# PRBonn/SHINE_mapping

Hardware: NVIDIA H100
Metric: sdf_train_points_per_sec_fwd_bwd (higher is better)
Workload: dtype f32

## Files before the change

shine_mapping_b200/csrc/shine_b200.cu:

```cuda

#include <cuda_runtime.h>
#include <math.h>
#include <stdint.h>

#include "shine_b200.h"

#ifndef SHINE_SECTOR_PROBE_TRAIN
#define SHINE_SECTOR_PROBE_TRAIN 0
#endif
#ifndef SHINE_SECTOR_PROBE_INFER
#define SHINE_SECTOR_PROBE_INFER 1
#endif
#ifndef SHINE_CPASYNC_PREFETCH
#define SHINE_CPASYNC_PREFETCH 0
#endif
#ifndef SHINE_GATHER_GROUP
#define SHINE_GATHER_GROUP 2
#endif
#ifndef SHINE_SLOT_PREFETCH
#define SHINE_SLOT_PREFETCH 0
#endif
#ifndef SHINE_ZERO_TILE_SKIP
#define SHINE_ZERO_TILE_SKIP 1
#endif
// ... 246 lines not shown
    const float s0 = odd ? v[0] : v[2], s1 = odd ? v[1] : v[3];
    const float r0 = __shfl_xor_sync(kFull, s0, 1), r1 = __shfl_xor_sync(kFull, s1, 1);
    if (!odd) { a[0] = v[0]; a[2] = v[1]; a[1] = r0; a[3] = r1; }
    else      { a[0] = r0;   a[2] = r1;   a[1] = v[2]; a[3] = v[3]; }
}
__device__ __forceinline__ void from_cfrag(const float (&c)[4], int odd, float (&v)[4]) {
    const float s0 = odd ? c[0] : c[2], s1 = odd ? c[1] : c[3];
    const float r0 = __shfl_xor_sync(kFull, s0, 1), r1 = __shfl_xor_sync(kFull, s1, 1);
    if (!odd) { v[0] = c[0]; v[1] = c[1]; v[2] = r0; v[3] = r1; }
    else      { v[0] = r0;   v[1] = r1;   v[2] = c[2]; v[3] = c[3]; }
}

#define SHINE_ACC_DECL float dW2[2][4][4], dW1[2][4], db2p[4][2], db1p[4][2], dw3p[4][2]

__device__ __forceinline__ float reduce_scatter_g8(const float (&v)[8], int lane) {
    float a[4], b[2];
    const bool b4 = (lane & 16) != 0, b3 = (lane & 8) != 0, b2 = (lane & 4) != 0;
#pragma unroll
    for (int i = 0; i < 4; ++i) a[i] = (b4 ? v[4 + i] : v[i]) + __shfl_xor_sync(kFull, b4 ? v[i] : v[4 + i], 16);
#pragma unroll
    for (int i = 0; i < 2; ++i) b[i] = (b3 ? a[2 + i] : a[i]) + __shfl_xor_sync(kFull, b3 ? a[i] : a[2 + i], 8);
    return (b2 ? b[1] : b[0]) + __shfl_xor_sync(kFull, b2 ? b[0] : b[1], 4);
}
__device__ __forceinline__ void round_bar(int id) { asm volatile("bar.sync %0, 128;" ::"r"(id) : "memory"); }

__device__ __forceinline__ int frag_chunk(int lane) { return lane ^ ((lane >> 2) & 6); }
template <int NTF>
__device__ __forceinline__ void load_afrag(const float* blk, int c, AFrag<NTF>& a) {
    const float4 v = *reinterpret_cast<const float4*>(blk + 4 * c);
    a.set_packed(v.x, v.y, v.z, v.w);
}
__device__ __forceinline__ void load_bfrag(const float* blk, int c, uint2& bh, uint2& bl) {
    const float2 v = *reinterpret_cast<const float2*>(blk + 2 * c);
    split_fast2(v.x, v.y, bh.x, bh.y, bl.x, bl.y);
}
__device__ __forceinline__ void stage_afrags(float* blk, const int (&sq)[2], const float (&c)[4][4]) {
#pragma unroll
    for (int mt = 0; mt < 2; ++mt)
#pragma unroll
        for (int q = 0; q < 2; ++q)
            *reinterpret_cast<float4*>(blk + 128 * mt + 4 * sq[q]) = make_float4(c[2 * mt][q], c[2 * mt + 1][q], c[2 * mt][2 + q], c[2 * mt + 1][2 + q]);
}
__device__ __forceinline__ int xfrag_word(int ks, int c) { return 64 * ks + 2 * (c ^ (8 * ks)); }
__device__ __forceinline__ void load_xfrag(const float* sx, int ks, int c, uint2& bh, uint2& bl) {
    const float2 v = *reinterpret_cast<const float2*>(sx + xfrag_word(ks, c));
    split_fast2(v.x, v.y, bh.x, bh.y, bl.x, bl.y);
}


constexpr int kGatherGroup = SHINE_GATHER_GROUP;

using shine_internal::StepParams;

struct SmemPlan {
    static constexpr int W1 = 0;
    static constexpr int W1T = W1 + 2 * kH * kF;
    static constexpr int W2 = W1T + 2 * kF * kWS;
    static constexpr int W2T = W2 + 2 * kH * kWS;
    static constexpr int B1 = W2T + 2 * kH * kWS;
    static constexpr int B2 = B1 + kH;
    static constexpr int W3 = B2 + kH;
    static constexpr int B3 = W3 + kH;
    static constexpr int GSCALE = B3 + 1;
    static constexpr int kDecGradFloats = kH * kF + kH + kH * kH + kH + kH + 1;
    static constexpr int RND = B3 + 4;
    static constexpr int PRE = RND + 8;
    static constexpr int kPrePerWarp = 5 * kTile;
    static constexpr int STAGE = PRE + 8 * kPrePerWarp;
    static constexpr int SA2 = 0;
    static constexpr int SB2 = SA2 + kTile * kH;
    static constexpr int SA1 = SB2 + kTile * kH;
    static constexpr int SX = SA1 + kTile * kH;
    static constexpr int kStagePerWarp = SX + kTile * kF;
    static constexpr int kGroupPerLevel = 4 * kTile;
};

constexpr int kMaxGroupedRuns = 6;

__device__ __forceinline__ void red_add_f2(float* p, float a, float b) {
    asm volatile("red.global.add.v2.f32 [%0], {%1,%2};" ::"l"(p), "f"(a), "f"(b) : "memory");
}
__device__ __forceinline__ int group_slot(int p) { return 4 * (p & 3) + (p >> 2); }

template <int LMAX>
__device__ __forceinline__ void grouped_scatter(const StepParams& P, int L, int tile, const float* __restrict__ pt,
                                                float* __restrict__ dtile, const float (&dxc)[4], int lane) {
    const int g = lane >> 2, t = lane & 3;
    *reinterpret_cast<float2*>(dtile + g * kF + 2 * t) = make_float2(dxc[0], dxc[1]);
    *reinterpret_cast<float2*>(dtile + (g + 8) * kF + 2 * t) = make_float2(dxc[2], dxc[3]);
    __syncwarp();
    uint2 bh[2], bl[2];
#pragma unroll
    for (int c = 0; c < 2; ++c)
        split_fast2(dtile[(8 * c + t) * kF + g], dtile[(8 * c + t + 4) * kF + g], bh[c].x, bh[c].y, bl[c].x, bl[c].y);
    const float sx = (g & 4) ? 1.f : -1.f, ox = (g & 4) ? 0.f : 1.f;
    const float sy = (g & 2) ? 1.f : -1.f, oy = (g & 2) ? 0.f : 1.f;
    const float sz = (g & 1) ? 1.f : -1.f, oz = (g & 1) ? 0.f : 1.f;
// ... 65 lines not shown
            a0.set(rid[0] == r ? w[0] : 0.f, rid[0] == r + 1 ? w[0] : 0.f, rid[1] == r ? w[1] : 0.f, rid[1] == r + 1 ? w[1] : 0.f);
            a1.set(rid[2] == r ? w[2] : 0.f, rid[2] == r + 1 ? w[2] : 0.f, rid[3] == r ? w[3] : 0.f, rid[3] == r + 1 ? w[3] : 0.f);
            float c0[4] = {0.f, 0.f, 0.f, 0.f}, c1[4] = {0.f, 0.f, 0.f, 0.f};
            mma3x2<3>(c0, c1, a0, a1, bh[0], bl[0], bh[1], bl[1]);
            if (v1 >= 0) {
                const int row = __ldg(slot_words + 16 * (int64_t)v1 + id_off);
                red_add_f2(gb + (int64_t)row * kF + 2 * t, c0[0] + c1[0], c0[1] + c1[1]);
            }
            if (v2 >= 0) {
                const int row = __ldg(slot_words + 16 * (int64_t)v2 + id_off);
                red_add_f2(gb + (int64_t)row * kF + 2 * t, c0[2] + c1[2], c0[3] + c1[3]);
            }
        }
    }
    __syncwarp();
}

template <int NTF, bool TRAIN, bool DEC_GRAD, int LMAX, bool GROUPED = false>
__global__ void __launch_bounds__(256, !TRAIN ? SHINE_INFER_MINB : (DEC_GRAD && !GROUPED) ? SHINE_TRAIN_DECGRAD_MINB : SHINE_TRAIN_MINB)
sdf_fused_kernel(const __grid_constant__ StepParams P) {
    static_assert(!GROUPED || TRAIN, "the grouped scatter belongs to the training kernels");
    static_assert(!DEC_GRAD || TRAIN, "decoder gradients belong to the training kernels");
    static_assert(SmemPlan::kStagePerWarp >= SmemPlan::kDecGradFloats, "a warp's staging area holds its partial decoder gradient");
    extern __shared__ __align__(16) float smem[];
    uint32_t* smu = reinterpret_cast<uint32_t*>(smem);
    const int tid = threadIdx.x, lane = tid & 31, warp = tid >> 5;
    const int g = lane >> 2, t = lane & 3, odd = t & 1, half = t >> 1;
    constexpr int kWarps = 8;

    for (int i = tid; i < kH * kF; i += blockDim.x) {
        const int nrow = i / kF, k = i % kF;
        uint32_t hi, lo; split_tf32(P.dec.w1[i], hi, lo);
        smu[SmemPlan::W1 + i] = hi; smu[SmemPlan::W1 + kH * kF + i] = lo;
        smu[SmemPlan::W1T + k * kWS + nrow] = hi; smu[SmemPlan::W1T + kF * kWS + k * kWS + nrow] = lo;
    }
    for (int i = tid; i < kH * kH; i += blockDim.x) {
        const int nrow = i / kH, k = i % kH;
        uint32_t hi, lo; split_tf32(P.dec.w2[i], hi, lo);
        smu[SmemPlan::W2 + nrow * kWS + k] = hi; smu[SmemPlan::W2 + kH * kWS + nrow * kWS + k] = lo;
        smu[SmemPlan::W2T + k * kWS + nrow] = hi; smu[SmemPlan::W2T + kH * kWS + k * kWS + nrow] = lo;
    }
    if (tid < kH) {
        smem[SmemPlan::B1 + tid] = P.dec.b1 ? P.dec.b1[tid] : 0.f;
        smem[SmemPlan::B2 + tid] = P.dec.b2 ? P.dec.b2[tid] : 0.f;
        smem[SmemPlan::W3 + tid] = P.dec.w3[tid];
    }
    if (tid == 0) {
        smem[SmemPlan::B3] = P.dec.b3 ? P.dec.b3[0] : 0.f;
        smem[SmemPlan::GSCALE] = P.loss_scale * ((TRAIN && P.d_loss) ? __ldg(P.d_loss) : 1.0f);
    }
    constexpr int kPark = LMAX <= 4 ? 16 : 32;
    constexpr int kIdPark = 4 * LMAX;
    __syncthreads();
    SHINE_ACC_DECL;
#pragma unroll
    for (int a = 0; a < 2; ++a) {
#pragma unroll
        for (int b = 0; b < 4; ++b) { dW2[a][b][0] = dW2[a][b][1] = dW2[a][b][2] = dW2[a][b][3] = 0.f; }
        dW1[a][0] = dW1[a][1] = dW1[a][2] = dW1[a][3] = 0.f;
    }
#pragma unroll
    for (int j = 0; j < 4; ++j) { db2p[j][0] = db2p[j][1] = db1p[j][0] = db1p[j][1] = dw3p[j][0] = dw3p[j][1] = 0.f; }
    float dW2acc[2][4] = {{0.f, 0.f, 0.f, 0.f}, {0.f, 0.f, 0.f, 0.f}}, dW1acc[4] = {0.f, 0.f, 0.f, 0.f};
    float dw3acc = 0.f, db2acc[2] = {0.f, 0.f}, db1acc[2] = {0.f, 0.f};
    constexpr bool kRounds = DEC_GRAD && GROUPED;

    constexpr bool kSectorProbe = TRAIN ? (SHINE_SECTOR_PROBE_TRAIN != 0) : (SHINE_SECTOR_PROBE_INFER != 0);
    constexpr bool kSlotPrefetch = TRAIN && !kSectorProbe && (SHINE_SLOT_PREFETCH != 0) && (SHINE_CPASYNC_PREFETCH == 0);
    constexpr bool kZeroSkip = (SHINE_ZERO_TILE_SKIP != 0) && (SHINE_CPASYNC_PREFETCH == 0);
    const bool poly = P.oct.poly_interp != 0;
    const int L = P.oct.num_levels;

    float db3p = 0.f;
    float loss_acc = 0.f;

    float* stage = smem + SmemPlan::STAGE + warp * SmemPlan::kStagePerWarp;
    float* stX = stage + SmemPlan::SX;
    const int kp = g >> 2, fc = frag_chunk(lane);
    const int sq[2] = {frag_chunk(8 * t + (g & 3)), frag_chunk(8 * t + 4 + (g & 3))};
    float* gpt = smem + SmemPlan::STAGE + (DEC_GRAD ? 8 * SmemPlan::kStagePerWarp : 0) +
                 warp * (LMAX * SmemPlan::kGroupPerLevel + (DEC_GRAD ? 0 : kTile * kF));
    float* gdx = DEC_GRAD ? stX : gpt + LMAX * SmemPlan::kGroupPerLevel;

    auto wgrad_round = [&](bool staged) {
        if (lane == 0) smu[SmemPlan::RND + warp] = staged ? 1u : 0u;
        round_bar(1 + 2 * (threadIdx.x >> 7));
        uint32_t present = 0;
#pragma unroll
        for (int v = 0; v < kWarps; ++v) present |= (smu[SmemPlan::RND + v] != 0u ? 1u : 0u) << v;
        const int mt = warp & 1, np = (warp >> 1) & 1, kh = warp >> 2;
#pragma unroll
        for (int i = 0; i < kWarps / 2; ++i) {
            const int v = 4 * kh + i;
            if (!((present >> v) & 1u)) continue;
            const float* s = smem + SmemPlan::STAGE + v * SmemPlan::kStagePerWarp;
#pragma unroll
            for (int ks = 0; ks < 2; ++ks) {
                uint2 bh[2], bl[2];
#pragma unroll
                for (int n = 0; n < 2; ++n) load_bfrag(s + SmemPlan::SB2 + (4 * ks + 2 * np + n) * 64, fc, bh[n], bl[n]);
                AFrag<NTF> a;
                const float4 av = *reinterpret_cast<const float4*>(s + SmemPlan::SA2 + (2 * ks + mt) * 128 + 4 * fc);
                a.set_packed(av.x, av.y, av.z, av.w);
                if (np == 0) { db2acc[0] += av.x + av.z; db2acc[1] += av.y + av.w; }
                mma3x2<NTF>(dW2acc[0], dW2acc[1], a, a, bh[0], bl[0], bh[1], bl[1]);
            }
        }
#pragma unroll
        for (int vv = 0; vv < 2; ++vv) {
            const int v = 2 * (warp >> 1) + vv;
            if (!((present >> v) & 1u)) continue;
            const float* s = smem + SmemPlan::STAGE + v * SmemPlan::kStagePerWarp;
#pragma unroll
            for (int ks = 0; ks < 2; ++ks) {
                uint2 bh, bl;
                load_xfrag(s + SmemPlan::SX, ks, fc, bh, bl);
                AFrag<NTF> a;
                const float4 av = *reinterpret_cast<const float4*>(s + SmemPlan::SA1 + (2 * ks + mt) * 128 + 4 * fc);
                a.set_packed(av.x, av.y, av.z, av.w);
                db1acc[0] += av.x + av.z; db1acc[1] += av.y + av.w;
                mma3<NTF>(dW1acc, a, bh, bl);
            }
        }
        round_bar(2 + 2 * (threadIdx.x >> 7));
    };

    const int warp_global = blockIdx.x * kWarps + warp;
    const int warp_stride = gridDim.x * kWarps;

    bool consecutive = true;
#pragma unroll
    for (int i = 1; i < LMAX; ++i)
        if (i < L && P.oct.lv[i].level != P.oct.lv[0].level - i) consecutive = false;

    unsigned long long skey0 = 0ull;
    int smine[LMAX / 2];
    uint4 skf[LMAX / 2];
#pragma unroll
    for (int j = 0; j < LMAX / 2; ++j) smine[j] = -1;
    auto stage_slots = [&](bool v, float sx, float sy, float sz) {
        skey0 = v ? morton_of(sx, sy, sz, P.oct.lv[0].level) : 0ull;
#pragma unroll
        for (int j = 0; j < LMAX / 2; ++j) {
            const int i = 2 * j + half;
            smine[j] = -1;
            if (i < L && v) {
                const shine_level& lv = P.oct.lv[i];
                const unsigned long long kq = consecutive ? (skey0 >> (3 * i)) : morton_of(sx, sy, sz, lv.level);
// ... 18 lines not shown

#if SHINE_CPASYNC_PREFETCH
    float* pre = smem + SmemPlan::PRE + warp * SmemPlan::kPrePerWarp;
    const uint32_t pre_s = (uint32_t)__cvta_generic_to_shared(pre);
    auto prefetch_inputs = [&](int tl) {
        if (tl < P.num_tiles) {
            const int64_t base = (int64_t)tl * kTile;
            const int64_t left = P.n - base;
            const int npts = left < kTile ? (int)left : kTile;
#pragma unroll
            for (int r = 0; r < 3; ++r) {
                const int wd = lane + 32 * r;
                const float* src = nullptr;
                if (wd < 48) { if (wd < 3 * npts) src = P.coord + 3 * base + wd; }
                else if (wd < 64) { if (P.label && wd - 48 < npts) src = P.label + base + (wd - 48); }
                else if (wd < 80) { if (P.weighted && wd - 64 < npts) src = P.weight + base + (wd - 64); }
                if (src) asm volatile("cp.async.ca.shared.global [%0], [%1], 4;" ::"r"(pre_s + 4u * (uint32_t)wd), "l"(src) : "memory");
            }
        }
        asm volatile("cp.async.commit_group;" ::: "memory");
    };
    prefetch_inputs(warp_global);

    for (int tile = warp_global; tile - (kRounds ? warp : 0) < P.num_tiles; tile += warp_stride) {
        const int64_t base = (int64_t)tile * kTile;
        const int64_t myp = base + g + 8 * odd;
        asm volatile("cp.async.wait_group 0;" ::: "memory");
        __syncwarp();
        const bool valid = myp < P.n;
        float x = 0.f, y = 0.f, z = 0.f, lab = 0.f, wgt = 1.f;
        if (valid) {
            const int lp = g + 8 * odd;
            x = pre[3 * lp]; y = pre[3 * lp + 1]; z = pre[3 * lp + 2];
            if (P.label) lab = pre[48 + lp];
            if (P.weighted) wgt = fabsf(pre[64 + lp]);
        }
        __syncwarp();
        prefetch_inputs(tile + warp_stride);

#else
    float nx = 0.f, ny = 0.f, nz = 0.f, nlab = 0.f, nwgt = 1.f;
    bool nvalid = false;
    auto prefetch_inputs = [&](int tl) {
        const int64_t p = (int64_t)tile_of(tl) * kTile + g + 8 * odd;
        nvalid = tl < P.num_tiles && p < P.n;
        if (nvalid) {
            nx = __ldg(P.coord + 3 * p); ny = __ldg(P.coord + 3 * p + 1); nz = __ldg(P.coord + 3 * p + 2);
            if (P.label) nlab = __ldg(P.label + p);
            if (P.weighted) nwgt = fabsf(__ldg(P.weight + p));
        }
    };
    prefetch_inputs(warp_global);
    if (kSlotPrefetch) stage_slots(nvalid, nx, ny, nz);

    int phase = kZeroSkip ? 0 : 1;
    bool advance = false, last_pass = false;
    float pred0 = 0.f, zsum = 0.f;
    auto bce_point = [&](float pv, float lb, float wg, float& li, float& dp) {
        const float zt = __fdividef(1.0f, 1.0f + __expf(-__fdividef(lb, P.sigma)));
        const float e = __expf(-fabsf(pv));
        li = fmaxf(pv, 0.f) - pv * zt + __logf(1.0f + e);
        dp = 0.f;
        if (TRAIN) {
            const float rs = __fdividef(1.0f, 1.0f + e);
            const float sg = pv >= 0.f ? rs : e * rs;
            dp = (sg - zt) * wg * smem[SmemPlan::GSCALE];
        }
    };
    const bool dynamic = (SHINE_DYNAMIC_TILES != 0) && !kRounds && P.tile_counter != nullptr;
    int next_tile = 0, pending = 0;
    if (dynamic && lane == 0) pending = atomicAdd(P.tile_counter, 1);
    for (int seq = warp_global;; seq = !advance ? seq : (dynamic ? next_tile : seq + warp_stride)) {
        if (last_pass) break;
        const int tile = tile_of(seq);
        if (phase == 1 && seq - (kRounds ? warp : 0) >= P.num_tiles) {
            if constexpr (kZeroSkip && DEC_GRAD) {
#pragma unroll
                for (int o = 16; o > 0; o >>= 1) zsum += __shfl_xor_sync(kFull, zsum, o);
                if (lane == 0) smem[SmemPlan::PRE + warp] = zsum;
                __syncthreads();
                if (!kRounds && warp != 0) break;
                float tot = 0.f;
#pragma unroll
                for (int w = 0; w < kWarps; ++w) tot += smem[SmemPlan::PRE + w];
                if (tot == 0.f) break;
                zsum = tot;
                phase = 2;
            } else {
                break;
            }
        }
        const bool virt = phase != 1;
        last_pass = phase == 2;
        advance = !virt;
        if (kRounds && phase == 2 && warp != 0) { wgrad_round(false); continue; }
        const int64_t base = (int64_t)tile * kTile;
        const int64_t myp = base + g + 8 * odd;
        const bool valid = virt ? false : nvalid;
        const float x = nx, y = ny, z = nz, lab = nlab, wgt = nwgt;
        if (!virt) {
            if (dynamic) {
                next_tile = warp_stride + __shfl_sync(kFull, pending, 0);
                prefetch_inputs(next_tile);
                if (lane == 0) pending = atomicAdd(P.tile_counter, 1);
            } else {
                prefetch_inputs(seq + warp_stride);
            }
        }

#endif
        float feat[4];
        float pk[kPark];
        float idp[kIdPark];
        uint32_t hitmask = 0;
        if constexpr (kSectorProbe) {
        {
            float acc[8] = {0.f, 0.f, 0.f, 0.f, 0.f, 0.f, 0.f, 0.f};
#pragma unroll
// ... 123 lines not shown
                    const float wz = half ? b.tz : b.uz;
                    const float w0 = __fmul_rn(__fmul_rn(b.ux, b.uy), wz), w1 = __fmul_rn(__fmul_rn(b.ux, b.ty), wz);
                    const float w2 = __fmul_rn(__fmul_rn(b.tx, b.uy), wz), w3 = __fmul_rn(__fmul_rn(b.tx, b.ty), wz);
                    blend4(acc, r0, r1, r2, r3, w0, w1, w2, w3);
                }
            }
#pragma unroll
            for (int q = 0; q < 4; ++q) {
                const float send = half ? acc[q] : acc[4 + q];
                const float recv = __shfl_xor_sync(kFull, send, 2);
                feat[q] = (half ? acc[4 + q] : acc[q]) + recv;
            }
        }
        }
#if !SHINE_CPASYNC_PREFETCH
        if (kZeroSkip && phase == 1 && __ballot_sync(kFull, hitmask != 0u) == 0u) {
            if (!TRAIN && P.mask && half == 0 && valid) P.mask[myp] = 0;
            if (P.pred && half == 0 && valid) P.pred[myp] = pred0;
            if (P.label != nullptr && valid) {
                float li, dpz;
                bce_point(pred0, lab, wgt, li, dpz);
                if (half == 0) { loss_acc += wgt * li; zsum += dpz; }
            }
            if (kRounds) wgrad_round(false);
            continue;
        }
#endif
        if (!TRAIN && P.mask) {
            bool present = false;
#pragma unroll
            for (int i = 0; i < LMAX; ++i) present = (i == P.mask_level) ? (((hitmask >> i) & 1u) != 0) : present;
            if (half == 0 && valid) P.mask[myp] = (uint8_t)present;
        }

        AFrag<NTF> ax;
        {
            float a[4]; to_afrag(feat, odd, a);
            ax.set(a[0], a[1], a[2], a[3]);
        }
        if (DEC_GRAD) {
#pragma unroll
            for (int q = 0; q < 4; ++q) stX[xfrag_word(kp, frag_chunk(16 * half + 4 * q + (g & 3))) + odd] = feat[q];
        }
        float h1[4][4];
        uint32_t m1 = 0;
        {
            uint2 bh[4], bl[4];
// ... 44 lines not shown
#pragma unroll
                for (int r = 0; r < 4; ++r) h2[j][r] = fmaxf(h2[j][r], 0.f);
            }
        }
        float w3a[4], w3b[4];
#pragma unroll
        for (int j = 0; j < 4; ++j) { w3a[j] = smem[SmemPlan::W3 + 8 * j + 2 * t]; w3b[j] = smem[SmemPlan::W3 + 8 * j + 2 * t + 1]; }
        float p0 = 0.f, p8 = 0.f;
#pragma unroll
        for (int j = 0; j < 4; ++j) {
            p0 = fmaf(h2[j][0], w3a[j], p0); p0 = fmaf(h2[j][1], w3b[j], p0);
            p8 = fmaf(h2[j][2], w3a[j], p8); p8 = fmaf(h2[j][3], w3b[j], p8);
        }
        p0 += __shfl_xor_sync(kFull, p0, 1); p0 += __shfl_xor_sync(kFull, p0, 2);
        p8 += __shfl_xor_sync(kFull, p8, 1); p8 += __shfl_xor_sync(kFull, p8, 2);
        const float b3 = smem[SmemPlan::B3];
        p0 += b3; p8 += b3;
        const float pown = odd ? p8 : p0;
#if !SHINE_CPASYNC_PREFETCH
        if (kZeroSkip && phase == 0) { pred0 = pown; phase = 1; continue; }
#endif
        if (P.pred && half == 0 && valid) P.pred[myp] = pown;

        if (P.label == nullptr) {
            if (kRounds) wgrad_round(false);
            continue;
        }

        float dpo = 0.f;
        if (valid) {
#if !SHINE_CPASYNC_PREFETCH
            float li;
            bce_point(pown, lab, wgt, li, dpo);
            if (half == 0) loss_acc += wgt * li;
#else
            const float zt = __fdividef(1.0f, 1.0f + __expf(-__fdividef(lab, P.sigma)));
            const float e = __expf(-fabsf(pown));
            const float li = fmaxf(pown, 0.f) - pown * zt + __logf(1.0f + e);
            if (half == 0) loss_acc += wgt * li;
            if (TRAIN) {
                const float rs = __fdividef(1.0f, 1.0f + e);
                const float sg = pown >= 0.f ? rs : e * rs;
                dpo = (sg - zt) * wgt * smem[SmemPlan::GSCALE];
            }
#endif
        }
        if (!TRAIN) continue;
#if !SHINE_CPASYNC_PREFETCH
        if (kZeroSkip && phase == 2) dpo = (g == 0 && odd == 0) ? zsum : 0.f;
#endif

        const float dpx = __shfl_xor_sync(kFull, dpo, 1);
        const float dp0 = odd ? dpx : dpo, dp8 = odd ? dpo : dpx;
        float dh2[4][4];
        float db2t[4][2], db1t[4][2], dw3t[4][2];
#pragma unroll
        for (int j = 0; j < 4; ++j) {
            dh2[j][0] = h2[j][0] > 0.f ? dp0 * w3a[j] : 0.f; dh2[j][1] = h2[j][1] > 0.f ? dp0 * w3b[j] : 0.f;
            dh2[j][2] = h2[j][2] > 0.f ? dp8 * w3a[j] : 0.f; dh2[j][3] = h2[j][3] > 0.f ? dp8 * w3b[j] : 0.f;
            if (DEC_GRAD) {
                dw3t[j][0] = dp0 * h2[j][0] + dp8 * h2[j][2];  dw3t[j][1] = dp0 * h2[j][1] + dp8 * h2[j][3];
                db2t[j][0] = dh2[j][0] + dh2[j][2];            db2t[j][1] = dh2[j][1] + dh2[j][3];
            }
        }
        if (DEC_GRAD) stage_afrags(stage + SmemPlan::SA2 + 256 * kp, sq, dh2);
        if (DEC_GRAD && t == 0) db3p += dp0 + dp8;

        float dh1[4][4];
        {
#pragma unroll
            for (int j = 0; j < 4; ++j) { dh1[j][0] = dh1[j][1] = dh1[j][2] = dh1[j][3] = 0.f; }
#pragma unroll
            for (int kk = 0; kk < 4; ++kk) {
                AFrag<NTF> a; a.set(dh2[kk][0], dh2[kk][2], dh2[kk][1], dh2[kk][3]);
                uint2 bh[4], bl[4];
#pragma unroll
                for (int j = 0; j < 4; ++j) {
                    const int off = (8 * j + g) * kWS + 8 * kk + 2 * t;
                    bh[j] = *reinterpret_cast<const uint2*>(smu + SmemPlan::W2T + off);
                    bl[j] = *reinterpret_cast<const uint2*>(smu + SmemPlan::W2T + kH * kWS + off);
                }
                mma3x4<NTF>(dh1, a, bh, bl);
            }
#pragma unroll
            for (int j = 0; j < 4; ++j) {
#pragma unroll
                for (int r = 0; r < 4; ++r) dh1[j][r] = ((m1 >> (4 * j + r)) & 1u) ? dh1[j][r] : 0.f;
                if (DEC_GRAD) { db1t[j][0] = dh1[j][0] + dh1[j][2]; db1t[j][1] = dh1[j][1] + dh1[j][3]; }
            }
            if (DEC_GRAD) stage_afrags(stage + SmemPlan::SA1 + 256 * kp, sq, dh1);
        }
        float dxc[4] = {0.f, 0.f, 0.f, 0.f};
        {
            float dxo[4] = {0.f, 0.f, 0.f, 0.f};
#pragma unroll
            for (int kk = 0; kk < 4; kk += 2) {
                AFrag<NTF> a0, a1;
                a0.set(dh1[kk][0], dh1[kk][2], dh1[kk][1], dh1[kk][3]);
                a1.set(dh1[kk + 1][0], dh1[kk + 1][2], dh1[kk + 1][1], dh1[kk + 1][3]);
                const int off = g * kWS + 8 * kk + 2 * t;
                const uint2 bh0 = *reinterpret_cast<const uint2*>(smu + SmemPlan::W1T + off);
                const uint2 bl0 = *reinterpret_cast<const uint2*>(smu + SmemPlan::W1T + kF * kWS + off);
                const uint2 bh1 = *reinterpret_cast<const uint2*>(smu + SmemPlan::W1T + off + 8);
                const uint2 bl1 = *reinterpret_cast<const uint2*>(smu + SmemPlan::W1T + kF * kWS + off + 8);
                mma3x2<NTF>(dxc, dxo, a0, a1, bh0, bl0, bh1, bl1);
            }
#pragma unroll
            for (int r = 0; r < 4; ++r) dxc[r] += dxo[r];
        }

        if (DEC_GRAD && !kRounds) {
#pragma unroll
            for (int j = 0; j < 4; ++j) {
                db2p[j][0] += db2t[j][0]; db2p[j][1] += db2t[j][1];
                db1p[j][0] += db1t[j][0]; db1p[j][1] += db1t[j][1];
                dw3p[j][0] += dw3t[j][0]; dw3p[j][1] += dw3t[j][1];
            }
            __syncwarp();
#pragma unroll
            for (int ks = 0; ks < 2; ++ks) {
                uint2 bh[4], bl[4];
#pragma unroll
                for (int nt = 0; nt < 4; ++nt) load_bfrag(stage + SmemPlan::SB2 + (4 * ks + nt) * 64, fc, bh[nt], bl[nt]);
#pragma unroll
                for (int mt = 0; mt < 2; ++mt) {
                    AFrag<NTF> a;
                    load_afrag(stage + SmemPlan::SA2 + (2 * ks + mt) * 128, fc, a);
                    mma3x4<NTF>(dW2[mt], a, bh, bl);
                }
            }
#pragma unroll
            for (int ks = 0; ks < 2; ++ks) {
                uint2 bh, bl;
                load_xfrag(stX, ks, fc, bh, bl);
                AFrag<NTF> a0, a1;
                load_afrag(stage + SmemPlan::SA1 + (2 * ks) * 128, fc, a0);
                load_afrag(stage + SmemPlan::SA1 + (2 * ks + 1) * 128, fc, a1);
                mma3x2<NTF>(dW1[0], dW1[1], a0, a1, bh, bl, bh, bl);
            }
            __syncwarp();
        }
        if (kRounds) {
            float cols[8];
#pragma unroll
            for (int j = 0; j < 4; ++j) { cols[2 * j] = dw3t[j][0]; cols[2 * j + 1] = dw3t[j][1]; }
            dw3acc += reduce_scatter_g8(cols, lane);
            wgrad_round(true);
        }

#if !SHINE_CPASYNC_PREFETCH
        if (kSlotPrefetch) stage_slots(nvalid, nx, ny, nz);
#endif
        if constexpr (GROUPED) {
            static_assert(!GROUPED || !kSectorProbe, "the grouped scatter reads the node slots of the level-split walk");
            grouped_scatter<LMAX>(P, L, tile, gpt, gdx, dxc, lane);
            continue;
        }
        float dx[4];
        from_cfrag(dxc, odd, dx);
        const float (&qk)[kPark] = pk;
        const float (&qid)[kIdPark] = idp;
#pragma unroll
        for (int i = 0; i < LMAX; ++i) {
            int ids[8];
#pragma unroll
            for (int k = 0; k < 4; ++k) {
                const int mine = __float_as_int(qid[4 * i + k]);
                const int other = __shfl_xor_sync(kFull, mine, 2);
                ids[2 * k] = half ? other : mine;
                ids[2 * k + 1] = half ? mine : other;
// ... 10 lines not shown
                for (int c = 0; c < 8; c += 2) {
                    float w[2];
                    f2_unpack(f2_mul(f2_pack(xy[c >> 1], xy[c >> 1]), zz), w[0], w[1]);
#pragma unroll
                    for (int k = 0; k < 2; ++k) {
                        const f2_t wk = f2_pack(w[k], w[k]);
                        float g0, g1, g2, g3;
                        f2_unpack(f2_mul(wk, dx01), g0, g1); f2_unpack(f2_mul(wk, dx23), g2, g3);
#if SHINE_EXPERIMENT_NO_RED
                        if (P.sigma == -12345.f)
#endif
                        red_add_f4(gb + (int64_t)ids[c + k] * kF, g0, g1, g2, g3);
                    }
                }
            }
        }
    }

    if (P.loss && P.label) {
#pragma unroll
        for (int o = 16; o > 0; o >>= 1) loss_acc += __shfl_xor_sync(kFull, loss_acc, o);
        if (lane == 0 && loss_acc != 0.f) atomicAdd(P.loss, loss_acc * P.loss_scale);
    }
    if (kRounds) {
        float* part = stage;
        constexpr int oB1 = 128, oB3 = 224, kParts = 225, oW2 = 256, kW2Block = 16 * 16;
#pragma unroll
        for (int n = 0; n < 2; ++n) {
            *reinterpret_cast<float2*>(part + oW2 + g * 16 + 8 * n + 2 * t) = make_float2(dW2acc[n][0], dW2acc[n][1]);
            *reinterpret_cast<float2*>(part + oW2 + (g + 8) * 16 + 8 * n + 2 * t) = make_float2(dW2acc[n][2], dW2acc[n][3]);
        }
        *reinterpret_cast<float2*>(part + g * kF + 2 * t) = make_float2(dW1acc[0], dW1acc[1]);
        *reinterpret_cast<float2*>(part + (g + 8) * kF + 2 * t) = make_float2(dW1acc[2], dW1acc[3]);
        part[oB1 + 2 * kH + 8 * (g >> 1) + 2 * t + (g & 1)] = dw3acc;
        {
            const int mt = warp & 1, np = (warp >> 1) & 1;
#pragma unroll
            for (int r = 0; r < 2; ++r) {
                float d1 = db1acc[r], d2 = db2acc[r];
#pragma unroll
                for (int o = 1; o < 4; o <<= 1) { d1 += __shfl_xor_sync(kFull, d1, o); d2 += __shfl_xor_sync(kFull, d2, o); }
                if (t == 0) {
                    part[oB1 + 16 * mt + g + 8 * r] = d1;           part[oB1 + 16 * (1 - mt) + g + 8 * r] = 0.f;
                    part[oB1 + kH + 16 * mt + g + 8 * r] = np == 0 ? d2 : 0.f;   part[oB1 + kH + 16 * (1 - mt) + g + 8 * r] = 0.f;
                }
            }
        }
#pragma unroll
        for (int o = 16; o > 0; o >>= 1) db3p += __shfl_xor_sync(kFull, db3p, o);
        if (lane == 0) part[oB3] = db3p;
        __syncthreads();
        constexpr int kVecEnd = 2 * oB1 + (kParts - oB1);
        for (int i = tid; i < kVecEnd + 4 * kW2Block; i += blockDim.x) {
            float v = 0.f;
            float* dst;
            if (i < 2 * oB1) {
                const int m = i / oB1, e = i % oB1;
#pragma unroll
                for (int c = 0; c < kWarps / 2; ++c) v += smem[SmemPlan::STAGE + (2 * c + m) * SmemPlan::kStagePerWarp + e];
                dst = P.dec.gw1 + 16 * m * kF + e;
            } else if (i >= kVecEnd) {
                const int b = (i - kVecEnd) / kW2Block, e = (i - kVecEnd) % kW2Block;
                const float* p0 = smem + SmemPlan::STAGE + b * SmemPlan::kStagePerWarp + oW2 + e;
                v = p0[0] + p0[4 * SmemPlan::kStagePerWarp];
                dst = P.dec.gw2 + (16 * (b & 1) + e / 16) * kH + 16 * (b >> 1) + e % 16;
            } else {
                const int e = i - oB1;
#pragma unroll
                for (int w = 0; w < kWarps; ++w) v += smem[SmemPlan::STAGE + w * SmemPlan::kStagePerWarp + e];
                if (e < oB1 + kH) dst = P.dec.gb1 ? P.dec.gb1 + (e - oB1) : nullptr;
                else if (e < oB1 + 2 * kH) dst = P.dec.gb2 ? P.dec.gb2 + (e - oB1 - kH) : nullptr;
                else if (e < oB3) dst = P.dec.gw3 + (e - oB1 - 2 * kH);
                else dst = P.dec.gb3;
            }
            if (v != 0.f && dst) atomicAdd(dst, v);
        }
    }
    if (DEC_GRAD && !kRounds) {
        float* part = stage;
        constexpr int oW1 = 0, oB1 = 256, oW2 = 288, oB2 = 1312, oW3 = 1344, oB3 = 1376;
        __syncwarp();
#pragma unroll
        for (int mt = 0; mt < 2; ++mt) {
#pragma unroll
            for (int nt = 0; nt < 4; ++nt) {
                *reinterpret_cast<float2*>(part + oW2 + (16 * mt + g) * kH + 8 * nt + 2 * t) = make_float2(dW2[mt][nt][0], dW2[mt][nt][1]);
                *reinterpret_cast<float2*>(part + oW2 + (16 * mt + g + 8) * kH + 8 * nt + 2 * t) = make_float2(dW2[mt][nt][2], dW2[mt][nt][3]);
            }
            *reinterpret_cast<float2*>(part + oW1 + (16 * mt + g) * kF + 2 * t) = make_float2(dW1[mt][0], dW1[mt][1]);
            *reinterpret_cast<float2*>(part + oW1 + (16 * mt + g + 8) * kF + 2 * t) = make_float2(dW1[mt][2], dW1[mt][3]);
        }
#pragma unroll
        for (int j = 0; j < 4; ++j) {
#pragma unroll
            for (int q = 0; q < 2; ++q) {
                float a = db1p[j][q], b = db2p[j][q], c = dw3p[j][q];
#pragma unroll
                for (int o = 4; o < 32; o <<= 1) {
                    a += __shfl_xor_sync(kFull, a, o); b += __shfl_xor_sync(kFull, b, o); c += __shfl_xor_sync(kFull, c, o);
                }
                if (g == 0) {
                    part[oB1 + 8 * j + 2 * t + q] = a;
                    part[oB2 + 8 * j + 2 * t + q] = b;
                    part[oW3 + 8 * j + 2 * t + q] = c;
                }
            }
        }
#pragma unroll
        for (int o = 16; o > 0; o >>= 1) db3p += __shfl_xor_sync(kFull, db3p, o);
        if (lane == 0) part[oB3] = db3p;
        __syncthreads();
        for (int i = tid; i < SmemPlan::kDecGradFloats; i += blockDim.x) {
            float v = 0.f;
#pragma unroll
            for (int w = 0; w < kWarps; ++w) v += smem[SmemPlan::STAGE + w * SmemPlan::kStagePerWarp + i];
            if (v == 0.f) continue;
            float* dst;
            if (i < oB1) dst = P.dec.gw1 + i;
            else if (i < oW2) dst = P.dec.gb1 ? P.dec.gb1 + (i - oB1) : nullptr;
            else if (i < oB2) dst = P.dec.gw2 + (i - oW2);
            else if (i < oW3) dst = P.dec.gb2 ? P.dec.gb2 + (i - oB2) : nullptr;
            else if (i < oB3) dst = P.dec.gw3 + (i - oW3);
            else dst = P.dec.gb3;
            if (dst) atomicAdd(dst, v);
        }
    }
}



struct TcPlan {
    static constexpr int A2H = 0;
    static constexpr int A2L = A2H + 16384;
    static constexpr int A1H = A2H;
    static constexpr int A1L = A2H + 4096;
    static constexpr int W1H = A2L + 16384;
    static constexpr int W1L = W1H + 1024;
    static constexpr int W2H = W1L + 1024;
// ... 260 lines not shown
        for (int64_t i = (n4 << 2) + threadIdx.x; i < T.numel; i += blockDim.x) {
            float gk = T.grad[i];
            if (T.weight_decay != 0.f) gk = fmaf(T.weight_decay, T.param[i], gk);
            const float m = T.exp_avg[i] + (gk - T.exp_avg[i]) * A.omb1;
            const float v = A.beta2 * T.exp_avg_sq[i] + A.omb2 * gk * gk;
            T.exp_avg[i] = m; T.exp_avg_sq[i] = v;
            T.param[i] -= step_size * (m / (sqrtf(v) / bc2_sqrt + A.eps));
            if (A.zero_grad) T.grad[i] = 0.f;
        }
    }
}


int check_decoder(const shine_decoder* d, const shine_octree* o) {
    if (!d) return SHINE_ERR_INVALID_ARG;
    if (d->in_dim != kF || d->hidden != kH || d->mlp_level != 2 || o->feature_dim != kF) return SHINE_ERR_UNSUPPORTED;
    if (!d->w1 || !d->w2 || !d->w3) return SHINE_ERR_INVALID_ARG;
    return SHINE_OK;
}

template <int NTF, bool TRAIN, bool DEC_GRAD, int LMAX, bool GROUPED = false>
int launch_fused_t(const StepParams& P, cudaStream_t st) {
    auto kern = sdf_fused_kernel<NTF, TRAIN, DEC_GRAD, LMAX, GROUPED>;
    const int smem_floats = SmemPlan::STAGE + (DEC_GRAD ? 8 * SmemPlan::kStagePerWarp : 0) +
                            (GROUPED ? 8 * (LMAX * SmemPlan::kGroupPerLevel + (DEC_GRAD ? 0 : kTile * kF)) : 0);
    const size_t smem_bytes = (size_t)smem_floats * sizeof(float);
    static int per_sm_by_dev[kMaxDevices] = {0};
    int& per_sm_cached = per_sm_by_dev[current_device()];
    cudaError_t e;
    if (per_sm_cached == 0) {
        e = cudaFuncSetAttribute(kern, cudaFuncAttributeMaxDynamicSharedMemorySize, (int)smem_bytes);
        if (e != cudaSuccess) return (int)e;
        e = cudaFuncSetAttribute(kern, cudaFuncAttributePreferredSharedMemoryCarveout, cudaSharedmemCarveoutMaxShared);
        if (e != cudaSuccess) return (int)e;
        int q = 1;
        e = cudaOccupancyMaxActiveBlocksPerMultiprocessor(&q, kern, 256, smem_bytes);
        if (e != cudaSuccess) return (int)e;
        cudaFuncAttributes fa;
        e = cudaFuncGetAttributes(&fa, kern);
        if (e != cudaSuccess) return (int)e;
        const int by_regs = fa.numRegs > 0 ? 65536 / (fa.numRegs * 256) : 1;
        const int by_smem = (int)((227 * 1024) / (smem_bytes + 1024));
        int own = by_regs < by_smem ? by_regs : by_smem;
        if (own > 8) own = 8;
        if (own > q) q = own;
        per_sm_cached = q < 1 ? 1 : q;
    }
    const int per_sm = per_sm_cached;
// ... 366 lines not shown
```

Baseline: 3.812 billion.

## Replace cross-warp weight-gradient rounds with per-warp dW2 accumulation in shared memory

In the grouped decoder-gradient training kernel, the cross-warp 'wgrad_round' scheme is removed. It used named barriers so that groups of warps cooperatively computed dW2/dW1 from every warp's staged activations. Each warp now keeps its own full dW2 partial in a private shared-memory block, rebuilding the dh2 fragment from staged dp values and ReLU bitmasks, and accumulates dW1 in registers. Removing the per-tile barriers also lets this kernel use dynamic tile scheduling. The cost is more shared memory per warp (a 32x32 partial per warp), an extra smem read-modify-write of that partial on every tile, and more redundant MMA work per warp.

Result: faster. 3.976 billion (median of 6 runs) (+4.3%).

```diff
diff --git a/shine_mapping_b200/csrc/shine_b200.cu b/shine_mapping_b200/csrc/shine_b200.cu
--- a/shine_mapping_b200/csrc/shine_b200.cu
+++ b/shine_mapping_b200/csrc/shine_b200.cu
@@ -292,7 +292,6 @@
     for (int i = 0; i < 2; ++i) b[i] = (b3 ? a[2 + i] : a[i]) + __shfl_xor_sync(kFull, b3 ? a[i] : a[2 + i], 8);
     return (b2 ? b[1] : b[0]) + __shfl_xor_sync(kFull, b2 ? b[0] : b[1], 4);
 }
-__device__ __forceinline__ void round_bar(int id) { asm volatile("bar.sync %0, 128;" ::"r"(id) : "memory"); }
 
 __device__ __forceinline__ int frag_chunk(int lane) { return lane ^ ((lane >> 2) & 6); }
 template <int NTF>
@@ -333,16 +332,19 @@
     static constexpr int B3 = W3 + kH;
     static constexpr int GSCALE = B3 + 1;
     static constexpr int kDecGradFloats = kH * kF + kH + kH * kH + kH + kH + 1;
-    static constexpr int RND = B3 + 4;
-    static constexpr int PRE = RND + 8;
+    static constexpr int PRE = B3 + 4;
     static constexpr int kPrePerWarp = 5 * kTile;
     static constexpr int STAGE = PRE + 8 * kPrePerWarp;
-    static constexpr int SA2 = 0;
-    static constexpr int SB2 = SA2 + kTile * kH;
+    static constexpr int SB2 = 0;
     static constexpr int SA1 = SB2 + kTile * kH;
     static constexpr int SX = SA1 + kTile * kH;
-    static constexpr int kStagePerWarp = SX + kTile * kF;
+    static constexpr int SA2 = SX + kTile * kF;
+    static constexpr int SDP = SA2;
+    static constexpr int kStagePerWarp = SA2 + kTile * kH;
+    static constexpr int kStageGrouped = SDP + 2 * kTile;
+    __host__ __device__ static constexpr int stage_per_warp(bool grouped) { return grouped ? kStageGrouped : kStagePerWarp; }
     static constexpr int kGroupPerLevel = 4 * kTile;
+    static constexpr int kW2Part = kH * kH;
 };
 
 constexpr int kMaxGroupedRuns = 6;
@@ -454,6 +456,11 @@
     static_assert(!GROUPED || TRAIN, "the grouped scatter belongs to the training kernels");
     static_assert(!DEC_GRAD || TRAIN, "decoder gradients belong to the training kernels");
     static_assert(SmemPlan::kStagePerWarp >= SmemPlan::kDecGradFloats, "a warp's staging area holds its partial decoder gradient");
+    static_assert(SmemPlan::kStageGrouped >= kH * kF + 3 * kH + 1, "a grouped warp's staging area holds its partial bias / dW1 gradients");
+    static_assert(!(GROUPED && DEC_GRAD) ||
+                      (SmemPlan::STAGE + 8 * (SmemPlan::kStageGrouped + LMAX * SmemPlan::kGroupPerLevel + SmemPlan::kW2Part)) * 4 + 1024 <=
+                          227 * 1024 / SHINE_TRAIN_MINB,
+                  "the grouped kernel's shared memory fits SHINE_TRAIN_MINB blocks/SM");
     extern __shared__ __align__(16) float smem[];
     uint32_t* smu = reinterpret_cast<uint32_t*>(smem);
     const int tid = threadIdx.x, lane = tid & 31, warp = tid >> 5;
@@ -493,9 +500,7 @@
     }
 #pragma unroll
     for (int j = 0; j < 4; ++j) { db2p[j][0] = db2p[j][1] = db1p[j][0] = db1p[j][1] = dw3p[j][0] = dw3p[j][1] = 0.f; }
-    float dW2acc[2][4] = {{0.f, 0.f, 0.f, 0.f}, {0.f, 0.f, 0.f, 0.f}}, dW1acc[4] = {0.f, 0.f, 0.f, 0.f};
-    float dw3acc = 0.f, db2acc[2] = {0.f, 0.f}, db1acc[2] = {0.f, 0.f};
-    constexpr bool kRounds = DEC_GRAD && GROUPED;
+    float dw3acc = 0.f, db2acc[2][2] = {{0.f, 0.f}, {0.f, 0.f}}, db1acc[2][2] = {{0.f, 0.f}, {0.f, 0.f}};
 
     constexpr bool kSectorProbe = TRAIN ? (SHINE_SECTOR_PROBE_TRAIN != 0) : (SHINE_SECTOR_PROBE_INFER != 0);
     constexpr bool kSlotPrefetch = TRAIN && !kSectorProbe && (SHINE_SLOT_PREFETCH != 0) && (SHINE_CPASYNC_PREFETCH == 0);
@@ -506,56 +511,19 @@
     float db3p = 0.f;
     float loss_acc = 0.f;
 
-    float* stage = smem + SmemPlan::STAGE + warp * SmemPlan::kStagePerWarp;
+    constexpr int kStage = SmemPlan::stage_per_warp(GROUPED);
+    float* stage = smem + SmemPlan::STAGE + warp * kStage;
     float* stX = stage + SmemPlan::SX;
     const int kp = g >> 2, fc = frag_chunk(lane);
     const int sq[2] = {frag_chunk(8 * t + (g & 3)), frag_chunk(8 * t + 4 + (g & 3))};
-    float* gpt = smem + SmemPlan::STAGE + (DEC_GRAD ? 8 * SmemPlan::kStagePerWarp : 0) +
+    float* gpt = smem + SmemPlan::STAGE + (DEC_GRAD ? 8 * kStage : 0) +
                  warp * (LMAX * SmemPlan::kGroupPerLevel + (DEC_GRAD ? 0 : kTile * kF));
     float* gdx = DEC_GRAD ? stX : gpt + LMAX * SmemPlan::kGroupPerLevel;
-
-    auto wgrad_round = [&](bool staged) {
-        if (lane == 0) smu[SmemPlan::RND + warp] = staged ? 1u : 0u;
-        round_bar(1 + 2 * (threadIdx.x >> 7));
-        uint32_t present = 0;
-#pragma unroll
-        for (int v = 0; v < kWarps; ++v) present |= (smu[SmemPlan::RND + v] != 0u ? 1u : 0u) << v;
-        const int mt = warp & 1, np = (warp >> 1) & 1, kh = warp >> 2;
-#pragma unroll
-        for (int i = 0; i < kWarps / 2; ++i) {
-            const int v = 4 * kh + i;
-            if (!((present >> v) & 1u)) continue;
-            const float* s = smem + SmemPlan::STAGE + v * SmemPlan::kStagePerWarp;
-#pragma unroll
-            for (int ks = 0; ks < 2; ++ks) {
-                uint2 bh[2], bl[2];
-#pragma unroll
-                for (int n = 0; n < 2; ++n) load_bfrag(s + SmemPlan::SB2 + (4 * ks + 2 * np + n) * 64, fc, bh[n], bl[n]);
-                AFrag<NTF> a;
-                const float4 av = *reinterpret_cast<const float4*>(s + SmemPlan::SA2 + (2 * ks + mt) * 128 + 4 * fc);
-                a.set_packed(av.x, av.y, av.z, av.w);
-                if (np == 0) { db2acc[0] += av.x + av.z; db2acc[1] += av.y + av.w; }
-                mma3x2<NTF>(dW2acc[0], dW2acc[1], a, a, bh[0], bl[0], bh[1], bl[1]);
-            }
-        }
-#pragma unroll
-        for (int vv = 0; vv < 2; ++vv) {
-            const int v = 2 * (warp >> 1) + vv;
-            if (!((present >> v) & 1u)) continue;
-            const float* s = smem + SmemPlan::STAGE + v * SmemPlan::kStagePerWarp;
-#pragma unroll
-            for (int ks = 0; ks < 2; ++ks) {
-                uint2 bh, bl;
-                load_xfrag(s + SmemPlan::SX, ks, fc, bh, bl);
-                AFrag<NTF> a;
-                const float4 av = *reinterpret_cast<const float4*>(s + SmemPlan::SA1 + (2 * ks + mt) * 128 + 4 * fc);
-                a.set_packed(av.x, av.y, av.z, av.w);
-                db1acc[0] += av.x + av.z; db1acc[1] += av.y + av.w;
-                mma3<NTF>(dW1acc, a, bh, bl);
-            }
-        }
-        round_bar(2 + 2 * (threadIdx.x >> 7));
-    };
+    float* w2p = smem + SmemPlan::STAGE + 8 * kStage + 8 * LMAX * SmemPlan::kGroupPerLevel + warp * SmemPlan::kW2Part;
+    if (DEC_GRAD && GROUPED) {
+#pragma unroll
+        for (int f = 0; f < 8; ++f) *reinterpret_cast<float4*>(w2p + 128 * f + 4 * lane) = make_float4(0.f, 0.f, 0.f, 0.f);
+    }
 
     const int warp_global = blockIdx.x * kWarps + warp;
     const int warp_stride = gridDim.x * kWarps;
@@ -620,7 +588,7 @@
     };
     prefetch_inputs(warp_global);
 
-    for (int tile = warp_global; tile - (kRounds ? warp : 0) < P.num_tiles; tile += warp_stride) {
+    for (int tile = warp_global; tile < P.num_tiles; tile += warp_stride) {
         const int64_t base = (int64_t)tile * kTile;
         const int64_t myp = base + g + 8 * odd;
         asm volatile("cp.async.wait_group 0;" ::: "memory");
@@ -665,19 +633,19 @@
             dp = (sg - zt) * wg * smem[SmemPlan::GSCALE];
         }
     };
-    const bool dynamic = (SHINE_DYNAMIC_TILES != 0) && !kRounds && P.tile_counter != nullptr;
+    const bool dynamic = (SHINE_DYNAMIC_TILES != 0) && P.tile_counter != nullptr;
     int next_tile = 0, pending = 0;
     if (dynamic && lane == 0) pending = atomicAdd(P.tile_counter, 1);
     for (int seq = warp_global;; seq = !advance ? seq : (dynamic ? next_tile : seq + warp_stride)) {
         if (last_pass) break;
         const int tile = tile_of(seq);
-        if (phase == 1 && seq - (kRounds ? warp : 0) >= P.num_tiles) {
+        if (phase == 1 && seq >= P.num_tiles) {
             if constexpr (kZeroSkip && DEC_GRAD) {
 #pragma unroll
                 for (int o = 16; o > 0; o >>= 1) zsum += __shfl_xor_sync(kFull, zsum, o);
                 if (lane == 0) smem[SmemPlan::PRE + warp] = zsum;
                 __syncthreads();
-                if (!kRounds && warp != 0) break;
+                if (warp != 0) break;
                 float tot = 0.f;
 #pragma unroll
                 for (int w = 0; w < kWarps; ++w) tot += smem[SmemPlan::PRE + w];
@@ -691,7 +659,6 @@
         const bool virt = phase != 1;
         last_pass = phase == 2;
         advance = !virt;
-        if (kRounds && phase == 2 && warp != 0) { wgrad_round(false); continue; }
         const int64_t base = (int64_t)tile * kTile;
         const int64_t myp = base + g + 8 * odd;
         const bool valid = virt ? false : nvalid;
@@ -861,7 +828,6 @@
                 bce_point(pred0, lab, wgt, li, dpz);
                 if (half == 0) { loss_acc += wgt * li; zsum += dpz; }
             }
-            if (kRounds) wgrad_round(false);
             continue;
         }
 #endif
@@ -952,10 +918,7 @@
 #endif
         if (P.pred && half == 0 && valid) P.pred[myp] = pown;
 
-        if (P.label == nullptr) {
-            if (kRounds) wgrad_round(false);
-            continue;
-        }
+        if (P.label == nullptr) continue;
 
         float dpo = 0.f;
         if (valid) {
@@ -993,7 +956,23 @@
                 db2t[j][0] = dh2[j][0] + dh2[j][2];            db2t[j][1] = dh2[j][1] + dh2[j][3];
             }
         }
-        if (DEC_GRAD) stage_afrags(stage + SmemPlan::SA2 + 256 * kp, sq, dh2);
+        if (DEC_GRAD && !GROUPED) stage_afrags(stage + SmemPlan::SA2 + 256 * kp, sq, dh2);
+        if (DEC_GRAD && GROUPED) {
+            uint32_t mg = 0, mg8 = 0;
+#pragma unroll
+            for (int j = 0; j < 4; ++j)
+#pragma unroll
+                for (int q = 0; q < 2; ++q) {
+                    mg |= (h2[j][q] > 0.f ? 1u : 0u) << (8 * j + 2 * t + q);
+                    mg8 |= (h2[j][2 + q] > 0.f ? 1u : 0u) << (8 * j + 2 * t + q);
+                }
+            mg |= __shfl_xor_sync(kFull, mg, 1); mg8 |= __shfl_xor_sync(kFull, mg8, 1);
+            mg |= __shfl_xor_sync(kFull, mg, 2); mg8 |= __shfl_xor_sync(kFull, mg8, 2);
+            if (t == 0) {
+                *reinterpret_cast<float2*>(stage + SmemPlan::SDP + 2 * g) = make_float2(dp0, __uint_as_float(mg));
+                *reinterpret_cast<float2*>(stage + SmemPlan::SDP + 2 * (g + 8)) = make_float2(dp8, __uint_as_float(mg8));
+            }
+        }
         if (DEC_GRAD && t == 0) db3p += dp0 + dp8;
 
         float dh1[4][4];
@@ -1039,7 +1018,7 @@
             for (int r = 0; r < 4; ++r) dxc[r] += dxo[r];
         }
 
-        if (DEC_GRAD && !kRounds) {
+        if (DEC_GRAD && !GROUPED) {
 #pragma unroll
             for (int j = 0; j < 4; ++j) {
                 db2p[j][0] += db2t[j][0]; db2p[j][1] += db2t[j][1];
@@ -1070,12 +1049,55 @@
             }
             __syncwarp();
         }
-        if (kRounds) {
+        if (DEC_GRAD && GROUPED) {
             float cols[8];
 #pragma unroll
             for (int j = 0; j < 4; ++j) { cols[2 * j] = dw3t[j][0]; cols[2 * j + 1] = dw3t[j][1]; }
             dw3acc += reduce_scatter_g8(cols, lane);
-            wgrad_round(true);
+            __syncwarp();
+#pragma unroll
+            for (int mt = 0; mt < 2; ++mt) {
+                const int n = 16 * mt + g;
+                const float wn = smem[SmemPlan::W3 + n], wn8 = smem[SmemPlan::W3 + n + 8];
+                float acc[4][4];
+#pragma unroll
+                for (int nt = 0; nt < 4; ++nt) {
+                    const float4 v = *reinterpret_cast<const float4*>(w2p + 128 * (4 * mt + nt) + 4 * lane);
+                    acc[nt][0] = v.x; acc[nt][1] = v.y; acc[nt][2] = v.z; acc[nt][3] = v.w;
+                }
+#pragma unroll
+                for (int ks = 0; ks < 2; ++ks) {
+                    uint2 bh[4], bl[4];
+#pragma unroll
+                    for (int nt = 0; nt < 4; ++nt) load_bfrag(stage + SmemPlan::SB2 + (4 * ks + nt) * 64, fc, bh[nt], bl[nt]);
+                    const float2 e0 = *reinterpret_cast<const float2*>(stage + SmemPlan::SDP + 2 * (4 * ks + t));
+                    const float2 e8 = *reinterpret_cast<const float2*>(stage + SmemPlan::SDP + 2 * (4 * ks + t + 8));
+                    const uint32_t k0 = __float_as_uint(e0.y), k8 = __float_as_uint(e8.y);
+                    const float ax = (k0 >> n) & 1u ? e0.x * wn : 0.f, ay = (k0 >> (n + 8)) & 1u ? e0.x * wn8 : 0.f;
+                    const float az = (k8 >> n) & 1u ? e8.x * wn : 0.f, aw = (k8 >> (n + 8)) & 1u ? e8.x * wn8 : 0.f;
+                    db2acc[mt][0] += ax + az; db2acc[mt][1] += ay + aw;
+                    AFrag<NTF> af;
+                    af.set_packed(ax, ay, az, aw);
+                    mma3x4<NTF>(acc, af, bh, bl);
+                }
+#pragma unroll
+                for (int nt = 0; nt < 4; ++nt)
+                    *reinterpret_cast<float4*>(w2p + 128 * (4 * mt + nt) + 4 * lane) = make_float4(acc[nt][0], acc[nt][1], acc[nt][2], acc[nt][3]);
+            }
+#pragma unroll
+            for (int ks = 0; ks < 2; ++ks) {
+                uint2 bh, bl;
+                load_xfrag(stX, ks, fc, bh, bl);
+                AFrag<NTF> a[2];
+#pragma unroll
+                for (int mt = 0; mt < 2; ++mt) {
+                    const float4 av = *reinterpret_cast<const float4*>(stage + SmemPlan::SA1 + (2 * ks + mt) * 128 + 4 * fc);
+                    db1acc[mt][0] += av.x + av.z; db1acc[mt][1] += av.y + av.w;
+                    a[mt].set_packed(av.x, av.y, av.z, av.w);
+                }
+                mma3x2<NTF>(dW1[0], dW1[1], a[0], a[1], bh, bl, bh, bl);
+            }
+            __syncwarp();
         }
 
 #if !SHINE_CPASYNC_PREFETCH
@@ -1132,61 +1154,48 @@
         for (int o = 16; o > 0; o >>= 1) loss_acc += __shfl_xor_sync(kFull, loss_acc, o);
         if (lane == 0 && loss_acc != 0.f) atomicAdd(P.loss, loss_acc * P.loss_scale);
     }
-    if (kRounds) {
+    if (DEC_GRAD && GROUPED) {
         float* part = stage;
-        constexpr int oB1 = 128, oB3 = 224, kParts = 225, oW2 = 256, kW2Block = 16 * 16;
-#pragma unroll
-        for (int n = 0; n < 2; ++n) {
-            *reinterpret_cast<float2*>(part + oW2 + g * 16 + 8 * n + 2 * t) = make_float2(dW2acc[n][0], dW2acc[n][1]);
-            *reinterpret_cast<float2*>(part + oW2 + (g + 8) * 16 + 8 * n + 2 * t) = make_float2(dW2acc[n][2], dW2acc[n][3]);
-        }
-        *reinterpret_cast<float2*>(part + g * kF + 2 * t) = make_float2(dW1acc[0], dW1acc[1]);
-        *reinterpret_cast<float2*>(part + (g + 8) * kF + 2 * t) = make_float2(dW1acc[2], dW1acc[3]);
-        part[oB1 + 2 * kH + 8 * (g >> 1) + 2 * t + (g & 1)] = dw3acc;
-        {
-            const int mt = warp & 1, np = (warp >> 1) & 1;
+        constexpr int oB1 = 256, oB2 = 288, oW3 = 320, oB3 = 352, kVec = 353;
+#pragma unroll
+        for (int mt = 0; mt < 2; ++mt) {
+            *reinterpret_cast<float2*>(part + (16 * mt + g) * kF + 2 * t) = make_float2(dW1[mt][0], dW1[mt][1]);
+            *reinterpret_cast<float2*>(part + (16 * mt + g + 8) * kF + 2 * t) = make_float2(dW1[mt][2], dW1[mt][3]);
 #pragma unroll
             for (int r = 0; r < 2; ++r) {
-                float d1 = db1acc[r], d2 = db2acc[r];
+                float d1 = db1acc[mt][r], d2 = db2acc[mt][r];
 #pragma unroll
                 for (int o = 1; o < 4; o <<= 1) { d1 += __shfl_xor_sync(kFull, d1, o); d2 += __shfl_xor_sync(kFull, d2, o); }
-                if (t == 0) {
-                    part[oB1 + 16 * mt + g + 8 * r] = d1;           part[oB1 + 16 * (1 - mt) + g + 8 * r] = 0.f;
-                    part[oB1 + kH + 16 * mt + g + 8 * r] = np == 0 ? d2 : 0.f;   part[oB1 + kH + 16 * (1 - mt) + g + 8 * r] = 0.f;
-                }
-            }
-        }
+                if (t == 0) { part[oB1 + 16 * mt + g + 8 * r] = d1; part[oB2 + 16 * mt + g + 8 * r] = d2; }
+            }
+        }
+        part[oW3 + 8 * (g >> 1) + 2 * t + (g & 1)] = dw3acc;
 #pragma unroll
         for (int o = 16; o > 0; o >>= 1) db3p += __shfl_xor_sync(kFull, db3p, o);
         if (lane == 0) part[oB3] = db3p;
         __syncthreads();
-        constexpr int kVecEnd = 2 * oB1 + (kParts - oB1);
-        for (int i = tid; i < kVecEnd + 4 * kW2Block; i += blockDim.x) {
+        for (int i = tid; i < kVec + kH * kH; i += blockDim.x) {
             float v = 0.f;
             float* dst;
-            if (i < 2 * oB1) {
-                const int m = i / oB1, e = i % oB1;
-#pragma unroll
-                for (int c = 0; c < kWarps / 2; ++c) v += smem[SmemPlan::STAGE + (2 * c + m) * SmemPlan::kStagePerWarp + e];
-                dst = P.dec.gw1 + 16 * m * kF + e;
-            } else if (i >= kVecEnd) {
-                const int b = (i - kVecEnd) / kW2Block, e = (i - kVecEnd) % kW2Block;
-                const float* p0 = smem + SmemPlan::STAGE + b * SmemPlan::kStagePerWarp + oW2 + e;
-                v = p0[0] + p0[4 * SmemPlan::kStagePerWarp];
-                dst = P.dec.gw2 + (16 * (b & 1) + e / 16) * kH + 16 * (b >> 1) + e % 16;
+            if (i < kVec) {
+#pragma unroll
+                for (int w = 0; w < kWarps; ++w) v += smem[SmemPlan::STAGE + w * kStage + i];
+                if (i < oB1) dst = P.dec.gw1 + i;
+                else if (i < oB2) dst = P.dec.gb1 ? P.dec.gb1 + (i - oB1) : nullptr;
+                else if (i < oW3) dst = P.dec.gb2 ? P.dec.gb2 + (i - oB2) : nullptr;
+                else if (i < oB3) dst = P.dec.gw3 + (i - oW3);
+                else dst = P.dec.gb3;
             } else {
-                const int e = i - oB1;
-#pragma unroll
-                for (int w = 0; w < kWarps; ++w) v += smem[SmemPlan::STAGE + w * SmemPlan::kStagePerWarp + e];
-                if (e < oB1 + kH) dst = P.dec.gb1 ? P.dec.gb1 + (e - oB1) : nullptr;
-                else if (e < oB1 + 2 * kH) dst = P.dec.gb2 ? P.dec.gb2 + (e - oB1 - kH) : nullptr;
-                else if (e < oB3) dst = P.dec.gw3 + (e - oB1 - 2 * kH);
-                else dst = P.dec.gb3;
+                const int e = i - kVec, r = e / kH, c = e % kH;
+                const int f = 128 * (4 * (r >> 4) + (c >> 3)) + 4 * (4 * (r & 7) + ((c & 7) >> 1)) + 2 * ((r >> 3) & 1) + (c & 1);
+#pragma unroll
+                for (int w = 0; w < kWarps; ++w) v += w2p[(w - warp) * SmemPlan::kW2Part + f];
+                dst = P.dec.gw2 + e;
             }
             if (v != 0.f && dst) atomicAdd(dst, v);
         }
     }
-    if (DEC_GRAD && !kRounds) {
+    if (DEC_GRAD && !GROUPED) {
         float* part = stage;
         constexpr int oW1 = 0, oB1 = 256, oW2 = 288, oB2 = 1312, oW3 = 1344, oB3 = 1376;
         __syncwarp();
@@ -1223,7 +1232,7 @@
         for (int i = tid; i < SmemPlan::kDecGradFloats; i += blockDim.x) {
             float v = 0.f;
 #pragma unroll
-            for (int w = 0; w < kWarps; ++w) v += smem[SmemPlan::STAGE + w * SmemPlan::kStagePerWarp + i];
+            for (int w = 0; w < kWarps; ++w) v += smem[SmemPlan::STAGE + w * kStage + i];
             if (v == 0.f) continue;
             float* dst;
             if (i < oB1) dst = P.dec.gw1 + i;
@@ -1530,8 +1539,8 @@
 template <int NTF, bool TRAIN, bool DEC_GRAD, int LMAX, bool GROUPED = false>
 int launch_fused_t(const StepParams& P, cudaStream_t st) {
     auto kern = sdf_fused_kernel<NTF, TRAIN, DEC_GRAD, LMAX, GROUPED>;
-    const int smem_floats = SmemPlan::STAGE + (DEC_GRAD ? 8 * SmemPlan::kStagePerWarp : 0) +
-                            (GROUPED ? 8 * (LMAX * SmemPlan::kGroupPerLevel + (DEC_GRAD ? 0 : kTile * kF)) : 0);
+    const int smem_floats = SmemPlan::STAGE + (DEC_GRAD ? 8 * SmemPlan::stage_per_warp(GROUPED) : 0) +
+                            (GROUPED ? 8 * (LMAX * SmemPlan::kGroupPerLevel + (DEC_GRAD ? SmemPlan::kW2Part : kTile * kF)) : 0);
     const size_t smem_bytes = (size_t)smem_floats * sizeof(float);
     static int per_sm_by_dev[kMaxDevices] = {0};
     int& per_sm_cached = per_sm_by_dev[current_device()];
```
